# scipopt/SCIP-SDP

Hardware: AMD Instinct MI355X
Metric: node-SDP solves/sec, dense block n x n with m vars (IPM iters/sec in iters_per_sec) (higher is better)
Workload: dtype f64

## Files before the change

### include/hipsdp_units.h

```cpp
#ifndef HIPSDP_UNITS_H
#define HIPSDP_UNITS_H

#include "hipsdp.h"

#ifdef __cplusplus
extern "C" {
#endif

HIPSDP_API int  hipsdp_dgemm_selfcheck(int device, int M, int N, int K, int layB, int batch, int splitk, int flags, double beta,
   int* used_v2, long long* ndiff);
HIPSDP_API int  hipsdp_pass_at_unit(int device, int R, long long E, const double* A, const double* coef, double sa, const double* add, int split,
   double* out, int* chunks);
HIPSDP_API int  hipsdp_dgemm_selfcheck2(int device, int M, int N, int K, int layB, int batch, int splitk, int flags, double alpha, double beta,
   int reps, int* used, long long* ndiff, double* ms_tile, double* ms_fast);
HIPSDP_API int  hipsdp_gram_plan_info(int device, int M, long long K, int nslab, int* no, int* nd, int* nitems, double* span);
HIPSDP_API int  hipsdp_gram_selfcheck(int device, int M, long long K, int reps, int* used, double* maxdiff, long long* nrepro, double* ms_tile,
   double* ms_gram);
HIPSDP_API int  hipsdp_dgemm_selfcheck3(int device, int M, int N, int K, int layB, int batch, int splitk, int flags, double alpha, double beta,
   int reps, int* used, long long* ndiff, double* maxdiff, long long* nrepro, double* ms_tile, double* ms_fast);
HIPSDP_API int  hipsdp_schur_dense(int device, int m1, int n, const double* A, const double* X, const double* Zinv, double* Mx,
   double ws_gbytes);
HIPSDP_API int  hipsdp_schur_w(int device, int m1, int n, const double* A, const double* X, const double* Z, double* Mx);
HIPSDP_API int  hipsdp_schur_shard_time(int device, int m1, int n, int nranks, int rank, int by_columns, int reps, double ws_gbytes, double* ms);
HIPSDP_API int  hipsdp_schur_var_share_time(int device, int m1, int n, int nranks, int rank, int cw, int reps, double* ms, double* a2a_bytes);
HIPSDP_API int  hipsdp_schur_sparse_unit(int device, int n, int m, long long nnz, const int* var, const int* row, const int* col,
   const double* val, const double* X, const double* Zinv, double* Mx);
HIPSDP_API int  hipsdp_mfma_peak(int device, double ms, double* tflops, double* ghz);
HIPSDP_API int  hipsdp_potrf(int device, int n, double* A, int* fail);
HIPSDP_API int  hipsdp_potrf_ex(int device, int n, double* A, int psd, int v1, double* dinv, int* regmask, int* fail);
HIPSDP_API int  hipsdp_potrs(int device, int n, const double* A, int nrhs, double* rhs);
HIPSDP_API int  hipsdp_trtri(int device, int n, const double* A, double* Linv);
HIPSDP_API int  hipsdp_lambda_min(int device, int n, const double* W, int steps, double* theta, double* resid);
HIPSDP_API int  hipsdp_lambda_min_scaled(int device, int n, const double* L, const double* D, int steps, double* theta, double* resid);
HIPSDP_API int  hipsdp_solve1_fits(int m, int q, int nblk, const int* ns);
HIPSDP_API int  hipsdp_solve1_class(int m, int nblk, const int* ns);

#ifdef __cplusplus
}
#endif

#endif
```

### scip-sdp_amd/binding.py

```python
import ctypes as C
import os
import numpy as np

_HERE = os.path.dirname(os.path.abspath(__file__))
LIBPATH = os.environ.get("HIPSDP_LIB", os.path.join(_HERE, "lib", "libhipsdp.so"))

STATUS_NAMES = {0: "optimal", 1: "dual_infeasible", 2: "dual_unbounded", 3: "both_infeasible", 4: "iterlimit",
                5: "numeric", 6: "timelimit", 7: "objlimit", -1: "unsolved"}


class Params(C.Structure):
    _fields_ = [("gaptol", C.c_double), ("feastol", C.c_double), ("infeastol", C.c_double), ("objlimit", C.c_double),
                ("timelimit", C.c_double), ("gamma", C.c_double), ("ws_gbytes", C.c_double), ("maxiter", C.c_int),
                ("verbose", C.c_int), ("lanczos_steps", C.c_int), ("settings", C.c_int), ("pabstol", C.c_double), ("preoptgap", C.c_double)]


class Info(C.Structure):
    _fields_ = [("status", C.c_int), ("iterations", C.c_int), ("pobj", C.c_double), ("dobj", C.c_double),
                ("pinf", C.c_double), ("dinf", C.c_double), ("dabs", C.c_double), ("gap", C.c_double), ("mu", C.c_double),
                ("tau", C.c_double), ("kappa", C.c_double), ("solve_seconds", C.c_double), ("schur_seconds", C.c_double),
                ("schur_flops", C.c_double), ("schur_calls", C.c_int), ("chol_fail", C.c_int), ("warm_started", C.c_int),
                ("settings_used", C.c_int), ("schur_flops_executed", C.c_double)]


# ... 307 lines not shown
    col = np.ascontiguousarray(col, dtype=np.int32); val = _f64(val)
    X = _f64(X); Zinv = _f64(Zinv)
    Mx = np.zeros((m + 1, m + 1))
    _chk(ulib().hipsdp_schur_sparse_unit(device, n, m, C.c_longlong(len(val)), _ip(var), _ip(row), _ip(col), _dp(val), _dp(X), _dp(Zinv), _dp(Mx)),
         "hipsdp_schur_sparse_unit")
    return Mx


def schur_w(A, X, Z, device=0):
    A = _f64(A)
    m1, n = A.shape[0], A.shape[1]
    X = _f64(X)
    Z = _f64(Z)
    Mx = np.zeros((m1, m1))
    _chk(ulib().hipsdp_schur_w(device, m1, n, _dp(A), _dp(X), _dp(Z), _dp(Mx)), "hipsdp_schur_w")
    return Mx


def dgemm_selfcheck(M, N, K, layB=1, batch=1, splitk=1, flags=0, beta=0.0, device=0):
    used = C.c_int(0)
    nd = C.c_longlong(0)
    _chk(ulib().hipsdp_dgemm_selfcheck(device, M, N, K, layB, batch, splitk, flags, C.c_double(beta), C.byref(used), C.byref(nd)),
         "hipsdp_dgemm_selfcheck")
    return used.value, nd.value


def dgemm_selfcheck2(M, N, K, layB=1, batch=1, splitk=1, flags=0, alpha=1.0, beta=0.0, reps=0, device=0):
    used = C.c_int(0)
    nd = C.c_longlong(0)
    t0, t1 = C.c_double(0.0), C.c_double(0.0)
    _chk(ulib().hipsdp_dgemm_selfcheck2(device, M, N, K, layB, batch, splitk, flags, C.c_double(alpha), C.c_double(beta), reps,
                                       C.byref(used), C.byref(nd), C.byref(t0), C.byref(t1)), "hipsdp_dgemm_selfcheck2")
    return used.value, nd.value, t0.value, t1.value


def dgemm_selfcheck3(M, N, K, layB=1, batch=1, splitk=1, flags=0, alpha=1.0, beta=0.0, reps=0, device=0):
    used = C.c_int(0)
    nd, nr = C.c_longlong(0), C.c_longlong(0)
    md, t0, t1 = C.c_double(0.0), C.c_double(0.0), C.c_double(0.0)
    _chk(ulib().hipsdp_dgemm_selfcheck3(device, M, N, K, layB, batch, splitk, flags, C.c_double(alpha), C.c_double(beta), reps,
                                       C.byref(used), C.byref(nd), C.byref(md), C.byref(nr), C.byref(t0), C.byref(t1)), "hipsdp_dgemm_selfcheck3")
    return used.value, nd.value, md.value, nr.value, t0.value, t1.value


def gram_selfcheck(M, K, reps=0, device=0):
    used = C.c_int(0)
    nr = C.c_longlong(0)
    md, t0, t1 = C.c_double(0.0), C.c_double(0.0), C.c_double(0.0)
    _chk(ulib().hipsdp_gram_selfcheck(device, M, C.c_longlong(K), reps, C.byref(used), C.byref(md), C.byref(nr), C.byref(t0), C.byref(t1)),
         "hipsdp_gram_selfcheck")
    return used.value, md.value, nr.value, t0.value, t1.value


def potrf(A, device=0):
    L = _f64(A).copy()
    fail = C.c_int(0)
    _chk(ulib().hipsdp_potrf(device, L.shape[0], _dp(L), C.byref(fail)), "hipsdp_potrf")
    return np.tril(L), fail.value


def potrf_ex(A, psd=False, v1=False, device=0):
    L = _f64(A).copy()
    n = L.shape[0]
    dinv = np.zeros(((n + 63) // 64) * 4096)
    mask = np.zeros(n, dtype=np.int32)
    fail = C.c_int(0)
    _chk(ulib().hipsdp_potrf_ex(device, n, _dp(L), int(psd), int(v1), _dp(dinv), _ip(mask), C.byref(fail)), "hipsdp_potrf_ex")
    return L, dinv, mask, fail.value


def potrs(A, rhs, device=0):
    A = _f64(A)
    r = _f64(rhs).copy()
    r2 = r.reshape(-1, A.shape[0])
    _chk(ulib().hipsdp_potrs(device, A.shape[0], _dp(A), r2.shape[0], _dp(r2)), "hipsdp_potrs")
    return r2.reshape(r.shape)


def trtri(A, device=0):
    A = _f64(A)
    Li = np.zeros_like(A)
    _chk(ulib().hipsdp_trtri(device, A.shape[0], _dp(A), _dp(Li)), "hipsdp_trtri")
    return Li


def lambda_min(W, steps=0, device=0):
    W = _f64(W)
    th = C.c_double(0.0)
    rs = C.c_double(0.0)
    _chk(ulib().hipsdp_lambda_min(device, W.shape[0], _dp(W), steps, C.byref(th), C.byref(rs)), "hipsdp_lambda_min")
    return th.value, rs.value


def syev(A, device=0):
    A = _f64(A)
    n = A.shape[0]
    lam = np.zeros(n)
    V = np.zeros((n, n))
    _chk(lib().hipsdp_syev(device, n, _dp(A), _dp(lam), _dp(V)), "hipsdp_syev")
    return lam, V


def gemv_n(A, V, device=0):
    A = _f64(A)
    V = _f64(V).reshape(-1, A.shape[1])
    out = np.zeros((V.shape[0], A.shape[0]))
# ... 26 lines not shown
```

### scip-sdp_amd/csrc/hs_kernels.h

```cpp
#ifndef HS_KERNELS_H
#define HS_KERNELS_H

#include "hs_common.h"

int hs_fill(hipStream_t s, double* p, long long n, double v);
int hs_set_identity(hipStream_t s, double* A, int n, double v);
int hs_copy(hipStream_t s, double* dst, const double* src, long long n);
int hs_axpy(hipStream_t s, long long n, double a, const double* x, double* y);
int hs_scale_add(hipStream_t s, long long n, double a, const double* x, double b, const double* y, double* out);
int hs_mirror_lower(hipStream_t s, double* A, int n, long long lda);
int hs_symmetrize(hipStream_t s, double* A, int n);
int hs_transpose(hipStream_t s, int n, const double* src, double* dst);

int hs_gemv_n(hipStream_t s, int R, long long E, const double* A, long long lda, int nv, const double* const* V,
   double* out, long long ldo, double* ws, long long wsdoubles);
int hs_gemv_t(hipStream_t s, int R, long long E, const double* A, long long lda, const double* coef, double sa,
   const double* add, double* out);

int hs_gemv_t_chunks(int R, long long E);
int hs_gemv_t_ws(hipStream_t s, int R, long long E, const double* A, long long lda, const double* coef, double sa,
   const double* add, double* out, double* ws, long long wsdoubles);
int hs_gemv_t3(hipStream_t s, int R, long long E, const double* A, long long lda, const double* c0, const double* c1, const double* c2,
   double* o0, double* o1, double* o2);

void hs_red_batch_begin(hipStream_t s);
int hs_red_batch_end(void);
int hs_red_batch_end_publish(hipStream_t s, int n, const double* src, double* dst, unsigned long long seq, unsigned long long* flag);
void hs_red_batch_reset(void);
int hs_fill_scalar(hipStream_t s, double* p, double v);
int hs_red_batch_solve(hipStream_t s, int m, const double* dinv, const double* L, int nrhs, double* vec, long long ld);
struct hs_rb_finish { int m; double eta, rg, sigmu, tau, kappa, etk; const double* u1; const double* u2; double* dy; double* dyt; double* sc;
   int s0, bub, bh, wrp, bu1, dtau, dkappa, den; };
int hs_red_batch_finish(hipStream_t s, const void* fin, size_t bytes);
int hs_copy_scalar(hipStream_t s, double* dst, const double* src);
void hs_red_batch_hold(hipStream_t s);
int hs_red_batch_release(void);
int hs_red_batch_flush(void);
int hs_red_batch_end_all(void);
int hs_make_ext(hipStream_t s, int m, double s0, double s1, const double* v, double* ext);
int hs_lp_rows_small(hipStream_t s, int q, int m1, const double* Dext, const double* v, int mode, double eta, double sigmu, const double* x,
   const double* z, const double* rd, const double* elp, double* out1, double* out2);
#define HS_AS_MAXBLK 8
struct hs_as_args { int nblk; int n2[HS_AS_MAXBLK]; const double* A[HS_AS_MAXBLK]; const double* V[HS_AS_MAXBLK]; };
int hs_apply_A_small(hipStream_t s, int m1, const hs_as_args* B, int q, const double* Dext, const double* vlp, double* out, int epi,
   double scal, const double* vin, double* vout);
int hs_axpy3(hipStream_t s, double a, long long n1, const double* x1, double* y1, long long n2, const double* x2, double* y2,
   long long n3, const double* x3, double* y3);
int hs_dot(hipStream_t s, long long n, const double* a, const double* b, double* out, int accumulate, double* ws);
int hs_absmax(hipStream_t s, long long n, const double* a, double* out, int accumulate, double* ws);
int hs_ratio_min(hipStream_t s, long long n, const double* x, const double* d, double* out, int accumulate, double* ws);

#define HS_SMALL_N 48
int hs_dir_block_small(hipStream_t s, int n, double c, const double* X, const double* R, const double* E, const double* Zinv,
   double s1, double* out);
int hs_dirmat(hipStream_t s, int n, double s1, const double* Zinv, const double* X, const double* GZ, double* H);

int hs_lp_dir(hipStream_t s, int q, double sigmu, double eta, const double* x, const double* z, const double* rd_or_dz,
   const double* elp, double* out);
int hs_lp_scale_rows(hipStream_t s, int q, int cols, const double* x, const double* z, const double* D, double* S);
int hs_vec_mul(hipStream_t s, long long n, const double* a, const double* b, double* out);
int hs_lp_s0(hipStream_t s, int q, const double* x, const double* z, const double* beta, double* out, int accumulate, double* ws);

int hs_pack_rows(hipStream_t s, int m1, int n, long long Lp, const double* A, double* Apk);
int hs_pack_weighted(hipStream_t s, int n, const double* V, double* pk);
int hs_unpack_sym(hipStream_t s, int n, const double* pk, double sa, const double* add, double* out);
int hs_zero_upper(hipStream_t s, double* A, int n);

struct hs_schur_ws
{
   double*   T;
   double*   U;
   double*   K;
   double*   V;
   long long capT, capV;
   long long chunk_cols;
   long long n2;
   long long kws_len;
   int       full;
   double*   U2;
   double*   V2;
   void*     evP[2];
   void*     evX[2];
   void*     ev_g2;
   int       (*after_g1)(void*);
   void*     after_g1_arg;
};
int  hs_schur_ws_alloc(hs_schur_ws* w, int m1, long long n2max, double budget_gb);
void hs_schur_ws_free(hs_schur_ws* w);
int  hs_schur_U(hipStream_t s, int m1, int n, const double* A, const double* X, const double* Zinv, double* Mx,
   hs_schur_ws* w, int j_begin, int j_end);
int  hs_schur_W(hipStream_t s, int m1, int n, const double* A, const double* R, const double* G, double* Mx, hs_schur_ws* w);
int  hs_schur_W_identity(hipStream_t s, int m1, int n, const double* A, double* Mx, hs_schur_ws* w);
int  hs_schur_W_identity_range(hipStream_t s, int m1, int n, const double* A, long long k0, long long k1, double* Mx, hs_schur_ws* w);

int  hs_schur_Urows(hipStream_t s, int m1, int n, const double* A, const double* X, const double* Zinv, double* Mx,
   hs_schur_ws* w, int r_begin, int r_end);
void hs_shard_rows(int m1, int nranks, int rank, int* chunk_rows, int* first_begin, int* second_begin);
int  hs_schur_Wcols(hipStream_t s, int m1, int n, const double* A, const double* R, const double* G, double* Mx, hs_schur_ws* w,
   int c0, int cw);
void hs_shard_cols(int m1, int n, int nranks, int rank, int* c_begin, int* c_width);
int  hs_schur_Wvar(hipStream_t s, void* comm, int rank, int nranks, int m1, int n, const double* A, const double* R, const double* G,
   double* Mx, hs_schur_ws* w, int c0, int cw);
int  hs_schur_ws_alloc_var(hs_schur_ws* w, int m1, int nranks, int n, int cwmax);
int  hs_schur_ws_alloc_var_overlap(hs_schur_ws* w);
int  hs_schur_Wvar_all(hipStream_t s, hipStream_t sc, void* comm, int rank, int nranks, int m1, int n, const double* A, const double* R,
   const double* G, double* Mx, hs_schur_ws* w, int cwmax, int overlap);
void hs_var_rows(int m1, int nranks, int rank, int* r0, int* r1);
void hs_var_wrows(int n, int nranks, int rank, int* q0, int* q1);
int  hs_alltoall(void* comm, const double* send, double* recv, const long long* cnt, hipStream_t stream);
int  hs_allreduce_sum(void* comm, double* buf, long long count, hipStream_t stream);
int  hs_mirror_upper(hipStream_t s, double* A, int n, long long lda);
int  hs_allgather_inplace(void* comm, double* buf, long long count_per_rank, int rank, hipStream_t stream);
int  hs_allgather(void* comm, const double* send, double* recv, long long count_per_rank, hipStream_t stream);

struct hs_sparse;
int  hs_sp_prefers_sparse(int n, int m, long long nnz);
int  hs_sp_build(hs_sparse** out, int n, int m, long long nnz, const int* var, const int* row, const int* col, const double* val);
void hs_sp_free(hs_sparse* sp);
long long hs_sp_nnz(const hs_sparse* sp);
int  hs_sp_apply_A(hipStream_t s, const hs_sparse* sp, const double* V, double* out_var1);
int  hs_sp_apply_AT(hipStream_t s, const hs_sparse* sp, const double* coef, double* out);
int  hs_sp_schur(hipStream_t s, const hs_sparse* sp, const double* X, const double* Zinv, double* Mx);
int  hs_sp_expand(hipStream_t s, const hs_sparse* sp, double* A);

int hs_potrf(hipStream_t s, int n, double* A, double* dinv, int* flag, const double* diag0);
long long hs_potrf_dinv_len(int n);
int hs_potrf_psd(hipStream_t s, int n, double* A, double* dinv, int* flag, const double* diag0, int* regmask, int set_flag);
int hs_trtri(hipStream_t s, int n, const double* L, const double* dinv, double* Linv, double* tmp);
int hs_potrf_small_ext_pair(hipStream_t s, int n, double* const* L, double* const* dinv, int* const* flag, const double* const* base,
   const double* const* dir, double alpha, double* const* Mout, double* const* Linv, double* const* Gram, int set_flag);
int hs_potrf_small_ext(hipStream_t s, int n, double* L, double* dinv, int* flag, const double* base, const double* dir, double alpha,
   double* Mout, double* Linv, double* Gram, int set_flag);
int hs_schur_small(hipStream_t s, int m1, int nblk, const int* n, const double* const* A, const double* const* X,
   const double* const* Zinv, int q, const double* Dext, const double* x, const double* z, double* Mx, double* Lm, double* diagM);
int hs_trsv(hipStream_t s, int n, const double* L, const double* dinv, int nrhs, double* rhs, long long ldr, int mode);
long long hs_trsv_sync_ws(int n);
int hs_trsv_sync_init(hipStream_t s, int n, int* sync_ws, int* epoch);
int hs_trsv_sync(hipStream_t s, int n, const double* L, const double* dinv, int nrhs, double* rhs, long long ldr, int mode,
   int* sync_ws, int* epoch);

int hs_lanczos_lmin(hipStream_t s, int n, const double* W, int maxsteps, double* res, double* ws);
long long hs_lanczos_ws(int n, int maxsteps);
#define HS_STEP_MAXJOBS 32
struct hs_step_jobs { int nblk; int n[HS_STEP_MAXJOBS]; const double* L0[HS_STEP_MAXJOBS]; const double* D0[HS_STEP_MAXJOBS];
   const double* L1[HS_STEP_MAXJOBS]; const double* D1[HS_STEP_MAXJOBS]; double* res0[HS_STEP_MAXJOBS]; double* res1[HS_STEP_MAXJOBS]; };
int hs_steplen_small_multi(hipStream_t s, const hs_step_jobs* P, int maxsteps);
// ... 313 lines not shown
```

### scip-sdp_amd/csrc/ipm.hip

```cpp
#include "hs_kernels.h"
#include "../../include/hipsdp.h"
#include <rocprofiler-sdk-roctx/roctx.h>
#include <vector>
#include <utility>
#include <functional>
#include <chrono>
#include <algorithm>
#include <cmath>
#include <cstdio>
#include <cstdlib>
#include <cstring>

#define HS_LAUNCH_CHECK() do { hipError_t e_ = hipGetLastError(); if ( e_ != hipSuccess ) { hs_record_hip_error(e_, "kernel launch", __FILE__, __LINE__); return HS_ERR_HIP; } } while (0)

enum
{
   SC_AX0 = 0,
   SC_DOBJ,
   SC_XZ,
   SC_RP2,
   SC_RD2,
   SC_RDLPMAX,
   SC_HP2,
   SC_HD2,
   SC_S0,
   SC_BUB,
   SC_BH,
   SC_WRP,
   SC_BU1,
   SC_DTAU,
   SC_DKAPPA,
   SC_RATX,
   SC_RATZ,
   SC_DEN,
   SC_FIXED_END = 24
};
#define SC_BLK(k, i) (SC_FIXED_END + 8 * (k) + (i))

struct Block
{
   int     n;
   double* A;
   double* Aown;
   double* A0;
   double* A0sep;
   double* Apkown;
   double *X, *Z, *Rd, *Lz, *LzInv, *Zinv, *Lx, *LxInv, *B, *H, *G, *GZ, *dXa, *dZa, *dX, *dZ, *E, *W, *T1;
   double *dinvz, *dinvx;
   double *Xs, *Zs;
   double *T2, *W2;
   double *Xpre;
   double *P2;
   double *pk3;
   double *Apk;
   double *pkv;
   long long Lp;
   bool apk_valid;
   bool derived_valid;
   bool sparse;
   bool sp_dirty;
   hs_sparse* sp;
// ... 3197 lines not shown
               if ( identity_start && it == 0 )
               {
                  if ( g == g0 )
                  {
                     const long long n2 = (long long) B.n * B.n;
                     const int G = s->comm != NULL ? s->nranks : 1, r = s->comm != NULL ? s->rank : 0;
                     const long long k0 = ((n2 * r / G) / 8) * 8, k1 = r == G - 1 ? n2 : ((n2 * (r + 1) / G) / 8) * 8;
                     HS_CALL( hs_schur_W_identity_range(st, m1, B.n, B.A, k0, k1, s->Mx, &s->sws) );
                  }
                  gram_only_used = true;
                  continue;
               }
               HS_CALL( hs_schur_Wcols(st, m1, B.n, B.A, B.Lx, B.LzInv, s->Mx, &s->sws, c0, cw) );
            }
         if ( s->comm != NULL )
            HS_CALL( hs_allreduce_sum(s->comm, s->Mx, (long long) m1 * m1, st) );
      }
      else if ( s->comm != NULL || s->schur_mode_rows )
      {
         int c, b1, b2;
         hs_shard_rows(m1, s->nranks, s->rank, &c, &b1, &b2);
         for (auto& B : s->blk)
         {
            if ( B.sparse )
               continue;
            HS_CALL( hs_schur_Urows(st, m1, B.n, B.A, B.X, B.Zinv, s->Mx, &s->sws, b1, b1 + c) );
            HS_CALL( hs_schur_Urows(st, m1, B.n, B.A, B.X, B.Zinv, s->Mx, &s->sws, b2, b2 + c) );
         }
         if ( s->comm != NULL )
         {
            const long long cnt = (long long) c * m1;
            HS_CALL( hs_allgather_inplace(s->comm, s->Mx, cnt, s->rank, st) );
            HS_CALL( hs_allgather(s->comm, s->Mx + (long long) b2 * m1, s->Mgather, cnt, st) );
            for (int r = 0; r < s->nranks; ++r)
            {
               const long long dstrow = (long long) (2 * s->nranks - 1 - r) * c;
               if ( dstrow >= m1 )
                  continue;
               long long rowsleft = m1 - dstrow;
               if ( rowsleft > c ) rowsleft = c;
               HS_CALL( hs_copy(st, s->Mx + dstrow * m1, s->Mgather + (long long) r * cnt, rowsleft * m1) );
            }
         }
         HS_CALL( hs_mirror_upper(st, s->Mx, m1, m1) );
      }
      else
      {
         for (auto& B : s->blk)
         {
            if ( B.sparse )
               continue;
            if ( identity_start && it == 0 )
            {
               HS_CALL( hs_schur_W_identity(st, m1, B.n, B.A, s->Mx, &s->sws) );
               gram_only_used = true;
            }
            else if ( s->schur_mode_U )
               HS_CALL( hs_schur_U(st, m1, B.n, B.A, B.X, B.Zinv, s->Mx, &s->sws, 0, m1) );
            else
               HS_CALL( hs_schur_W(st, m1, B.n, B.A, B.Lx, B.LzInv, s->Mx, &s->sws) );
         }
      }
      for (auto& B : s->blk)
      {
         if ( !B.sparse )
            continue;
         const int n = B.n;
         HS_CALL( gemm(s, HS_KC, HS_MC, n, n, n, 1.0, B.X, n, B.A0, n, 0.0, B.T1, n) );
         HS_CALL( gemm(s, HS_KC, HS_MC, n, n, n, 1.0, B.T1, n, B.Zinv, n, 0.0, B.W, n) );
         HS_CALL( pass_A(s, B, B.W, s->tmpe) );
         hipLaunchKernelGGL(k_add_col0, g1d(m1), dim3(256), 0, st, m1, s->tmpe, s->Mx);
         HS_LAUNCH_CHECK();
         HS_CALL( hs_sp_schur(st, B.sp, B.X, B.Zinv, s->Mx) );
      }
      if ( q > 0 )
      {
         HS_CALL( hs_lp_scale_rows(st, q, m1, s->x, s->z, s->Dext, s->Slp) );
         HS_CALL( gemm(s, HS_MC, HS_MC, m1, m1, q, 1.0, s->Dext, m1, s->Slp, m1, 1.0, s->Mx, m1, HS_GEMM_LOWER) );
      }
      return hs_mirror_lower(st, s->Mx, m1, m1);
   }

   int solve_m()
   {
      phase_mark(s, PH_MSOLVE);
      predH_queued = predH_joined = split_dz = false;
      if ( s->use2 && s->comm == NULL && !small_problem(s) && m > 0 )
      {
         HS_CALL( fork2(s) );
         {
            QueueSwap sw(s);
            HS_CALL( direction(s, 0.0, 1.0, mu, rg, false, 0.0, 1) );
         }
         predH_queued = true;
      }
      if ( m > 0 )
      {
         if ( !schur_small )
         {
            HS_HIP( hipMemcpy2DAsync(s->Lm, (size_t) m * sizeof(double), s->Mx + m1 + 1, (size_t) m1 * sizeof(double),
                  (size_t) m * sizeof(double), (size_t) m, hipMemcpyDeviceToDevice, st) );
            HS_HIP( hipMemcpy2DAsync(s->dya, sizeof(double), s->Mx + m1 + 1, (size_t) (m1 + 1) * sizeof(double), sizeof(double), (size_t) m,
                  hipMemcpyDeviceToDevice, st) );
         }
         HS_CALL( hs_potrf_psd(st, m, s->Lm, s->dinvm, s->flags + 2, s->dya, s->regmask, setf) );
         if ( m <= 64 )
         {
// ... 965 lines not shown
```

### scip-sdp_amd/csrc/kernels.hip

```cpp
#include "hs_kernels.h"
#include <string.h>
#include <stdio.h>
#include <stdlib.h>

static int hs_rec_dir_block_small(hipStream_t s, int n, double c, const double* X, const double* R, const double* E, const double* Zinv,
   double s1, double* out);
static int hs_rec_lp_dir(hipStream_t s, int q, double sigmu, double eta, const double* x, const double* z, const double* r, const double* elp,
   double* out);
static int hs_rec_vec_mul(hipStream_t s, long long n, const double* a, const double* b, double* out);
static int hs_rec_axpy3(hipStream_t s, double a, long long n1, const double* x1, double* y1, long long n2, const double* x2, double* y2,
   long long n3, const double* x3, double* y3);
static int hs_rec_gemv_t(hipStream_t s, int R, long long E, const double* A, long long lda, const double* coef, double sa, const double* add,
   double* out);

struct __attribute__((aligned(16))) dbl2 { double x, y; };
__device__ __forceinline__ dbl2 load_stream2(const double* p)
{
   typedef double gv2 __attribute__((ext_vector_type(2)));
   const gv2 t = __builtin_nontemporal_load(reinterpret_cast<const gv2*>(p));
   dbl2 r; r.x = t.x; r.y = t.y;
   return r;
}

static inline int hs_launch_ok(void)
// ... 21 lines not shown
   }
}

__global__ void k_scale_add(long long n, double a, const double* __restrict__ x, double b, const double* __restrict__ y,
   double* __restrict__ out)
{
   for (long long i = (long long) blockIdx.x * blockDim.x + threadIdx.x; i < n; i += (long long) gridDim.x * blockDim.x)
   {
      double v = a * x[i];
      if ( y != NULL )
         v += b * y[i];
      out[i] = v;
   }
}

__global__ void k_mirror_lower(double* A, int n, long long lda)
{
   const long long total = (long long) n * n;
   for (long long i = (long long) blockIdx.x * blockDim.x + threadIdx.x; i < total; i += (long long) gridDim.x * blockDim.x)
   {
      const int r = (int) (i / n);
      const int c = (int) (i - (long long) r * n);
      if ( r < c )
         A[(long long) r * lda + c] = A[(long long) c * lda + r];
   }
}

__global__ void k_mirror_upper(double* A, int n, long long lda)
{
   const long long total = (long long) n * n;
   for (long long i = (long long) blockIdx.x * blockDim.x + threadIdx.x; i < total; i += (long long) gridDim.x * blockDim.x)
   {
      const int r = (int) (i / n);
      const int c = (int) (i - (long long) r * n);
      if ( r > c )
         A[(long long) r * lda + c] = A[(long long) c * lda + r];
   }
}

__global__ void k_pack_rows(int m1, int n, long long Lp, const double* __restrict__ A, double* __restrict__ Apk)
{
   const long long n2 = (long long) n * n;
   const long long total = (long long) m1 * n2;
   for (long long e = (long long) blockIdx.x * blockDim.x + threadIdx.x; e < total; e += (long long) gridDim.x * blockDim.x)
   {
      const long long i = e / n2;
      const long long rc = e - i * n2;
      const int r = (int) (rc / n), c = (int) (rc - (long long) r * n);
      if ( c <= r )
         Apk[i * Lp + (long long) r * (r + 1) / 2 + c] = A[e];
   }
}

__global__ void k_pack_weighted(int n, const double* __restrict__ V, double* __restrict__ pk)
{
   const long long total = (long long) n * n;
   for (long long e = (long long) blockIdx.x * blockDim.x + threadIdx.x; e < total; e += (long long) gridDim.x * blockDim.x)
   {
      const int r = (int) (e / n), c = (int) (e - (long long) (e / n) * n);
      if ( c <= r )
         pk[(long long) r * (r + 1) / 2 + c] = (r == c ? 1.0 : 2.0) * V[e];
   }
}

__global__ void k_unpack_sym(int n, const double* __restrict__ pk, double sa, const double* __restrict__ add, double* __restrict__ out)
{
   const long long total = (long long) n * n;
   for (long long e = (long long) blockIdx.x * blockDim.x + threadIdx.x; e < total; e += (long long) gridDim.x * blockDim.x)
   {
      const int r0 = (int) (e / n), c0 = (int) (e - (long long) (e / n) * n);
      const int r = r0 > c0 ? r0 : c0, c = r0 > c0 ? c0 : r0;
      double v = pk[(long long) r * (r + 1) / 2 + c];
      if ( add != NULL )
         v += sa * add[e];
      out[e] = v;
   }
}

__global__ void k_zero_upper(double* A, int n)
{
   const long long total = (long long) n * n;
   for (long long i = (long long) blockIdx.x * blockDim.x + threadIdx.x; i < total; i += (long long) gridDim.x * blockDim.x)
   {
      const int r = (int) (i / n);
      const int c = (int) (i - (long long) r * n);
      if ( r < c )
         A[i] = 0.0;
   }
}

__global__ void k_symmetrize(double* A, int n)
{
   const long long total = (long long) n * n;
   for (long long i = (long long) blockIdx.x * blockDim.x + threadIdx.x; i < total; i += (long long) gridDim.x * blockDim.x)
   {
      const int r = (int) (i / n);
      const int c = (int) (i - (long long) r * n);
      if ( r > c )
      {
         const double v = 0.5 * (A[(long long) r * n + c] + A[(long long) c * n + r]);
         A[(long long) r * n + c] = v;
         A[(long long) c * n + r] = v;
      }
   }
}

// ... 103 lines not shown

int hs_axpy3(hipStream_t s, double a, long long n1, const double* x1, double* y1, long long n2, const double* x2, double* y2,
   long long n3, const double* x3, double* y3)
{
   if ( n1 < 0 ) n1 = 0;
   if ( n2 < 0 ) n2 = 0;
   if ( n3 < 0 ) n3 = 0;
   if ( n1 + n2 + n3 == 0 ) return HS_OK;
   if ( hs_rec_axpy3(s, a, n1, x1, y1, n2, x2, y2, n3, x3, y3) )
      return HS_OK;
   hipLaunchKernelGGL(k_axpy3, dim3(grid_for(n1 + n2 + n3, 256, 2048)), dim3(256), 0, s, a, n1, x1, y1, n2, x2, y2, n3, x3, y3);
   HS_LAUNCH_CHECK();
   return HS_OK;
}

int hs_scale_add(hipStream_t s, long long n, double a, const double* x, double b, const double* y, double* out)
{
   (void) hs_red_batch_flush();
   if ( n <= 0 ) return HS_OK;
   hipLaunchKernelGGL(k_scale_add, dim3(grid_for(n, 256, 2048)), dim3(256), 0, s, n, a, x, b, y, out);
   HS_LAUNCH_CHECK();
   return HS_OK;
}

int hs_axpy(hipStream_t s, long long n, double a, const double* x, double* y)
{
   (void) hs_red_batch_flush();
   return hs_scale_add(s, n, a, x, 1.0, y, y);
}

int hs_mirror_lower(hipStream_t s, double* A, int n, long long lda)
{
   (void) hs_red_batch_flush();
   if ( n <= 1 ) return HS_OK;
   hipLaunchKernelGGL(k_mirror_lower, dim3(grid_for((long long) n * n, 256, 2048)), dim3(256), 0, s, A, n, lda);
   HS_LAUNCH_CHECK();
   return HS_OK;
}

int hs_mirror_upper(hipStream_t s, double* A, int n, long long lda)
{
   (void) hs_red_batch_flush();
   if ( n <= 1 ) return HS_OK;
   hipLaunchKernelGGL(k_mirror_upper, dim3(grid_for((long long) n * n, 256, 2048)), dim3(256), 0, s, A, n, lda);
   HS_LAUNCH_CHECK();
   return HS_OK;
}

int hs_pack_rows(hipStream_t s, int m1, int n, long long Lp, const double* A, double* Apk)
{
   (void) hs_red_batch_flush();
   HS_HIP( hipMemsetAsync(Apk, 0, (size_t) m1 * (size_t) Lp * sizeof(double), s) );
   hipLaunchKernelGGL(k_pack_rows, dim3(grid_for((long long) m1 * n * n, 256, 65536)), dim3(256), 0, s, m1, n, Lp, A, Apk);
   HS_LAUNCH_CHECK();
   return HS_OK;
}

int hs_pack_weighted(hipStream_t s, int n, const double* V, double* pk)
{
   (void) hs_red_batch_flush();
   hipLaunchKernelGGL(k_pack_weighted, dim3(grid_for((long long) n * n, 256, 2048)), dim3(256), 0, s, n, V, pk);
   HS_LAUNCH_CHECK();
   return HS_OK;
}

int hs_unpack_sym(hipStream_t s, int n, const double* pk, double sa, const double* add, double* out)
{
   (void) hs_red_batch_flush();
   hipLaunchKernelGGL(k_unpack_sym, dim3(grid_for((long long) n * n, 256, 2048)), dim3(256), 0, s, n, pk, sa, add, out);
   HS_LAUNCH_CHECK();
   return HS_OK;
}

int hs_zero_upper(hipStream_t s, double* A, int n)
{
   (void) hs_red_batch_flush();
   if ( n <= 1 ) return HS_OK;
   hipLaunchKernelGGL(k_zero_upper, dim3(grid_for((long long) n * n, 256, 2048)), dim3(256), 0, s, A, n);
   HS_LAUNCH_CHECK();
   return HS_OK;
}

__global__ void __launch_bounds__(256) k_transpose(int n, const double* __restrict__ src, double* __restrict__ dst)
{
   __shared__ double tile[32][33];
   const int bx = blockIdx.x * 32, by = blockIdx.y * 32;
   const int tx = threadIdx.x & 31, ty = threadIdx.x >> 5;
   for (int r = ty; r < 32; r += 8)
      if ( by + r < n && bx + tx < n )
         tile[r][tx] = src[(long long) (by + r) * n + bx + tx];
   __syncthreads();
   for (int r = ty; r < 32; r += 8)
      if ( bx + r < n && by + tx < n )
         dst[(long long) (bx + r) * n + by + tx] = tile[tx][r];
}

int hs_transpose(hipStream_t s, int n, const double* src, double* dst)
{
   (void) hs_red_batch_flush();
   if ( n <= 0 ) return HS_OK;
   const int t = (n + 31) / 32;
   hipLaunchKernelGGL(k_transpose, dim3(t, t), dim3(256), 0, s, n, src, dst);
   HS_LAUNCH_CHECK();
   return HS_OK;
}

// ... 1710 lines not shown
```

### scip-sdp_amd/csrc/schur.hip

```cpp
#include "hs_kernels.h"
#include "hs_lds_product.h"
#include <vector>
#include <cmath>
#include <stdlib.h>

int hs_schur_ws_alloc(hs_schur_ws* w, int m1, long long n2max, double budget_gb)
{
   w->T = w->U = w->K = w->V = w->U2 = w->V2 = NULL;
   w->evP[0] = w->evP[1] = w->evX[0] = w->evX[1] = NULL;
   w->ev_g2 = NULL;
   w->after_g1 = NULL; w->after_g1_arg = NULL;
   w->capT = w->capV = 0;
   const double need_full = 2.0 * 8.0 * (double) m1 * (double) n2max;
   long long cols = m1;
   w->full = 1;
   if ( need_full > budget_gb * 1e9 )
   {
      w->full = 0;
      cols = (long long) (budget_gb * 1e9 / (2.0 * 8.0 * (double) n2max));
      cols = (cols / 128) * 128;
      if ( cols < 128 ) cols = 128;
      if ( cols > m1 ) cols = m1;
   }
   w->chunk_cols = cols;
// ... 17 lines not shown
   w->kws_len = (long long) sk * m1 * (w->full ? m1 : cols);
   e = hs_pool_alloc((void**) &w->K, (size_t) w->kws_len * sizeof(double)) == HS_OK ? hipSuccess : hipErrorOutOfMemory;
   if ( e != hipSuccess )
   {
      hs_record_hip_error(e, "hipMalloc(split-K slabs)", __FILE__, __LINE__);
      return e == hipErrorOutOfMemory ? HS_ERR_NOMEM : HS_ERR_HIP;
   }
   return HS_OK;
}

void hs_schur_ws_free(hs_schur_ws* w)
{
   hs_pool_free(w->T);
   hs_pool_free(w->U);
   hs_pool_free(w->K);
   hs_pool_free(w->V);
   hs_pool_free(w->U2);
   hs_pool_free(w->V2);
   for (int i = 0; i < 2; ++i)
   {
      if ( w->evP[i] != NULL ) (void) hipEventDestroy((hipEvent_t) w->evP[i]);
      if ( w->evX[i] != NULL ) (void) hipEventDestroy((hipEvent_t) w->evX[i]);
      w->evP[i] = w->evX[i] = NULL;
   }
   w->T = w->U = w->K = w->V = w->U2 = w->V2 = NULL;
}

int hs_schur_U(hipStream_t s, int m1, int n, const double* A, const double* X, const double* Zinv, double* Mx,
   hs_schur_ws* w, int j_begin, int j_end)
{
   const long long n2 = (long long) n * n;
   if ( n2 > 2000000000LL )
      return HS_ERR_ARG;
   for (int j0 = j_begin; j0 < j_end; j0 += (int) w->chunk_cols)
   {
      const int cj = (j_end - j0) < w->chunk_cols ? (j_end - j0) : (int) w->chunk_cols;
      const long long rows = (long long) cj * n;
      if ( rows > 2000000000LL )
         return HS_ERR_ARG;
      hs_gemm_args g1 = {(int) rows, n, n, HS_KC, HS_MC, A + (long long) j0 * n2, n, 0, Zinv, n, 0, w->T, n, 0, 1.0, 0.0, 1, HS_GEMM_REMAP, 1, NULL};
      HS_CALL( hs_dgemm(s, &g1) );
      hs_gemm_args g2 = {n, n, n, HS_KC, HS_MC, X, n, 0, w->T, n, n2, w->U, n, n2, 1.0, 0.0, cj, HS_GEMM_REMAP, 1, NULL};
      HS_CALL( hs_dgemm(s, &g2) );
      const int rowsM = m1 - j0;
      int sk = hs_dgemm_pick_splitk(rowsM, cj, (int) n2, 1);
      while ( sk > 1 && (long long) sk * rowsM * cj > w->kws_len ) --sk;
      hs_gemm_args g3 = {rowsM, cj, (int) n2, HS_KC, HS_KC, A + (long long) j0 * n2, n2, 0, w->U, n2, 0,
         Mx + (long long) j0 * m1 + j0, m1, 0, 1.0, 1.0, 1, HS_GEMM_LOWER, sk, w->K};
      HS_CALL( hs_dgemm(s, &g3) );
   }
   return HS_OK;
}

static int schur_gram(hipStream_t s, int m1, long long K, const double* V, long long ldv, double* Mx, hs_schur_ws* w, int* done)
{
   *done = 0;
   long long nslab = w->kws_len / ((long long) m1 * m1);
   if ( nslab > 64 ) nslab = 64;
   double executed = 0.0;
   const int r = hs_gram_try(s, m1, K, V, ldv, Mx, m1, 1.0, 1.0, w->K, (int) nslab, &executed);
   if ( r < 0 )
      return -r;
   if ( r == 1 )
   {
      hs_mfma_flops_add(executed);
      *done = 1;
   }
   return HS_OK;
}

#define SYRK_MIN_M1 256

static void schur_syrk_shape(const hs_schur_ws* w, int m1, long long K, bool xcd, int* flags, int* sk)
{
   const long long slab = (long long) m1 * m1;
   *flags = HS_GEMM_LOWER;
   if ( xcd && 2 * slab <= w->kws_len )
   {
      const long long tm = (m1 + 127) / 128;
      int s = hs_dgemm_pick_xcd_slices(tm * (tm + 1) / 2, K);
      if ( s < 2 ) s = 2;
      while ( s > 2 && (long long) s * slab > w->kws_len ) --s;
      *sk = s;
      *flags |= HS_GEMM_XCD | HS_GEMM_NOFAST;
      return;
   }
   int s = hs_dgemm_pick_splitk(m1, m1, (int) K, 1);
   while ( s > 1 && (long long) s * slab > w->kws_len ) --s;
   *sk = s < 1 ? 1 : s;
}

int hs_schur_W_identity_range(hipStream_t s, int m1, int n, const double* A, long long k0, long long k1, double* Mx, hs_schur_ws* w)
{
   const long long n2 = (long long) n * n;
   const long long K = k1 - k0;
   if ( n2 > 2000000000LL || k0 < 0 || k1 > n2 || (k0 & 1) )
      return HS_ERR_ARG;
   if ( K <= 0 )
      return HS_OK;
   {
      int done = 0;
      HS_CALL( schur_gram(s, m1, K, A + k0, n2, Mx, w, &done) );
      if ( done )
         return HS_OK;
   }
   int flags, sk;
   schur_syrk_shape(w, m1, K, m1 >= SYRK_MIN_M1 && K >= 16384 && (K >= 50000 || m1 >= 900), &flags, &sk);
   hs_gemm_args g3 = {m1, m1, (int) K, HS_KC, HS_KC, A + k0, n2, 0, A + k0, n2, 0, Mx, m1, 0, 1.0, 1.0, 1, flags, sk, sk > 1 ? w->K : NULL};
   return hs_dgemm(s, &g3);
}

int hs_schur_W_identity(hipStream_t s, int m1, int n, const double* A, double* Mx, hs_schur_ws* w)
{
   return hs_schur_W_identity_range(s, m1, n, A, 0, (long long) n * n, Mx, w);
}

int hs_schur_W(hipStream_t s, int m1, int n, const double* A, const double* R, const double* G, double* Mx, hs_schur_ws* w)
{
   const long long n2 = (long long) n * n;
   const long long rows = (long long) m1 * n;
   if ( !w->full || n2 > 2000000000LL || rows > 2000000000LL )
      return HS_ERR_ARG;
   hs_gemm_args g1 = {(int) rows, n, n, HS_KC, HS_MC, A, n, 0, R, n, 0, w->T, n, 0, 1.0, 0.0, 1, HS_GEMM_B_LOWTRI, 1, NULL};
   HS_CALL( hs_dgemm(s, &g1) );
   if ( w->after_g1 != NULL )
   {
      int (*f)(void*) = w->after_g1;
      w->after_g1 = NULL;
      HS_CALL( f(w->after_g1_arg) );
   }
   if ( w->ev_g2 != NULL )
      HS_HIP( hipStreamWaitEvent(s, (hipEvent_t) w->ev_g2, 0) );
   hs_gemm_args g2 = {n, n, n, HS_KC, HS_MC, G, n, 0, w->T, n, n2, w->U, n, n2, 1.0, 0.0, m1, HS_GEMM_A_LOWTRI | HS_GEMM_REMAP, 1, NULL};
   HS_CALL( hs_dgemm(s, &g2) );
   {
      int done = 0;
      HS_CALL( schur_gram(s, m1, n2, w->U, n2, Mx, w, &done) );
      if ( done )
         return HS_OK;
   }
   int flags = HS_GEMM_LOWER;
   int sk;
   if ( m1 >= SYRK_MIN_M1 && n2 >= 16384 && (n2 >= 50000 || m1 >= 900) )
   {
      const long long tm = (m1 + 127) / 128;
      const long long ntri = tm * (tm + 1) / 2;
      sk = hs_dgemm_pick_xcd_slices(ntri, n2);
      while ( sk > 2 && (long long) sk * m1 * m1 > w->kws_len ) --sk;
      flags |= HS_GEMM_XCD;
      flags |= HS_GEMM_NOFAST;
   }
   else
   {
      sk = hs_dgemm_pick_splitk(m1, m1, (int) n2, 1);
      while ( sk > 1 && (long long) sk * m1 * m1 > w->kws_len ) --sk;
   }
   hs_gemm_args g3 = {m1, m1, (int) n2, HS_KC, HS_KC, w->U, n2, 0, w->U, n2, 0, Mx, m1, 0, 1.0, 1.0, 1, flags, sk, w->K};
   HS_CALL( hs_dgemm(s, &g3) );
   return HS_OK;
}

int hs_schur_Wcols(hipStream_t s, int m1, int n, const double* A, const double* R, const double* G, double* Mx, hs_schur_ws* w,
   int c0, int cw)
{
   if ( cw <= 0 )
      return HS_OK;
   const long long rows = (long long) m1 * n;
// ... 434 lines not shown
```

### scip-sdp_amd/csrc/units.hip

```cpp
#include "hs_kernels.h"
#include "../../include/hipsdp.h"
#include "../../include/hipsdp_units.h"
#include <vector>
#include <cstring>
#include <cstdlib>

namespace {

struct DevBuf
{
   double* p;
   DevBuf() : p(NULL) {}
   ~DevBuf() { if ( p ) (void) hipFree(p); }
   int alloc(long long n) { if ( n <= 0 ) n = 1; hipError_t e = hipMalloc((void**) &p, (size_t) n * sizeof(double)); if ( e != hipSuccess ) { hs_record_hip_error(e, "hipMalloc", __FILE__, __LINE__); return e == hipErrorOutOfMemory ? HS_ERR_NOMEM : HS_ERR_HIP; } return HS_OK; }
   int up(const double* h, long long n) { if ( n <= 0 ) return HS_OK; hipError_t e = hipMemcpy(p, h, (size_t) n * sizeof(double), hipMemcpyHostToDevice); if ( e != hipSuccess ) { hs_record_hip_error(e, "H2D", __FILE__, __LINE__); return HS_ERR_HIP; } return HS_OK; }
   int down(double* h, long long n) { if ( n <= 0 ) return HS_OK; hipError_t e = hipMemcpy(h, p, (size_t) n * sizeof(double), hipMemcpyDeviceToHost); if ( e != hipSuccess ) { hs_record_hip_error(e, "D2H", __FILE__, __LINE__); return HS_ERR_HIP; } return HS_OK; }
};

int pick_device(int device)
{
   int nd = 0;
   if ( hipGetDeviceCount(&nd) != hipSuccess || nd <= 0 )
      return HIPSDP_ERR_NODEVICE;
   if ( device < 0 || device >= nd )
// ... 261 lines not shown
   }
   *used = r2 == 1 ? 1 : 0;
   *maxdiff = 0.0; *nrepro = 0;
   unsigned long long h[2] = {0, 0};
   if ( rc == HS_OK && r2 == 1 )
   {
      if ( hipMemset(dn, 0, 2 * sizeof(unsigned long long)) != hipSuccess ) rc = HS_ERR_HIP;
      hipLaunchKernelGGL(k_unit_lowdiff, dim3(1024), dim3(256), 0, 0, M, dC1.p, dC2.p, dn);
      if ( rc == HS_OK && hipMemcpy(h, dn, sizeof(h), hipMemcpyDeviceToHost) != hipSuccess ) rc = HS_ERR_HIP;
      memcpy(maxdiff, &h[0], sizeof(double));
      if ( rc == HS_OK && hipMemset(dn, 0, 2 * sizeof(unsigned long long)) != hipSuccess ) rc = HS_ERR_HIP;
      hipLaunchKernelGGL(k_unit_lowdiff, dim3(1024), dim3(256), 0, 0, M, dC2.p, dC3.p, dn);
      if ( rc == HS_OK && hipMemcpy(h, dn, sizeof(h), hipMemcpyDeviceToHost) != hipSuccess ) rc = HS_ERR_HIP;
      *nrepro = (long long) h[1];
   }
   if ( rc == HS_OK && reps > 0 && ms_tile != NULL && ms_gram != NULL )
   {
      hipEvent_t e0, e1;
      HS_HIP( hipEventCreate(&e0) ); HS_HIP( hipEventCreate(&e1) );
      for (int which = 0; which < 2 && rc == HS_OK; ++which)
      {
         for (int it = -2; it < reps && rc == HS_OK; ++it)
         {
            if ( it == 0 )
               (void) hipEventRecord(e0, 0);
            if ( which == 0 )
               rc = hs_dgemm(0, &g3);
            else if ( r2 == 1 )
            {
               const int r = hs_gram_try(0, M, K, dW.p, K, dC2.p, M, 1.0, 1.0, dS.p, nslab, &ex);
               if ( r < 0 ) rc = -r;
            }
         }
         (void) hipEventRecord(e1, 0);
         float t = 0.f;
         if ( rc == HS_OK && (hipEventSynchronize(e1) != hipSuccess || hipEventElapsedTime(&t, e0, e1) != hipSuccess) )
            rc = HS_ERR_HIP;
         *(which == 0 ? ms_tile : ms_gram) = (double) t / reps;
      }
      (void) hipEventDestroy(e0); (void) hipEventDestroy(e1);
   }
   if ( rc == HS_OK && hipDeviceSynchronize() != hipSuccess )
      rc = HS_ERR_HIP;
   (void) hipFree(dn);
   return rc;
}

extern "C" int hipsdp_gram_plan_info(int device, int M, long long K, int nslab, int* no, int* nd, int* nitems, double* span)
{
   HS_CALL( pick_device(device) );
   return hs_gram_plan_info(M, K, nslab, no, nd, nitems, span) ? HIPSDP_OK : HIPSDP_ERR_ARG;
}

extern "C" int hipsdp_schur_dense(int device, int m1, int n, const double* A, const double* X, const double* Zinv, double* Mx,
   double ws_gbytes)
{
   HS_CALL( pick_device(device) );
   const long long n2 = (long long) n * n;
   DevBuf dA, dX, dZ, dM;
   HS_CALL( dA.alloc(m1 * n2) ); HS_CALL( dX.alloc(n2) ); HS_CALL( dZ.alloc(n2) ); HS_CALL( dM.alloc((long long) m1 * m1) );
   HS_CALL( dA.up(A, m1 * n2) ); HS_CALL( dX.up(X, n2) ); HS_CALL( dZ.up(Zinv, n2) );
   hs_schur_ws w;
   HS_CALL( hs_schur_ws_alloc(&w, m1, n2, ws_gbytes > 0.0 ? ws_gbytes : 1e9) );
   if ( ws_gbytes > 0.0 && w.chunk_cols > 1 )
   {
      long long cols = (long long) (ws_gbytes * 1e9 / (16.0 * (double) n2));
      if ( cols < 1 ) cols = 1;
      if ( cols < w.chunk_cols ) w.chunk_cols = cols;
   }
   HS_CALL( hs_fill(0, dM.p, (long long) m1 * m1, 0.0) );
   int rc = hs_schur_U(0, m1, n, dA.p, dX.p, dZ.p, dM.p, &w, 0, m1);
   if ( rc == HS_OK ) rc = hs_mirror_lower(0, dM.p, m1, m1);
   if ( rc == HS_OK && hipDeviceSynchronize() != hipSuccess ) rc = HS_ERR_HIP;
   hs_schur_ws_free(&w);
   HS_CALL( rc );
   HS_CALL( dM.down(Mx, (long long) m1 * m1) );
   return HIPSDP_OK;
}

extern "C" int hipsdp_schur_shard_time(int device, int m1, int n, int nranks, int rank, int by_columns, int reps, double ws_gbytes,
   double* ms)
{
   HS_CALL( pick_device(device) );
   if ( m1 < 1 || n < 1 || nranks < 1 || rank < 0 || rank >= nranks || reps < 1 || ms == NULL )
      return HIPSDP_ERR_ARG;
   const long long n2 = (long long) n * n;
   DevBuf dA, dX, dZ, dM;
   HS_CALL( dA.alloc(m1 * n2) ); HS_CALL( dX.alloc(n2) ); HS_CALL( dZ.alloc(n2) ); HS_CALL( dM.alloc((long long) (m1 + 32) * m1) );
   hipLaunchKernelGGL(k_unit_fill, dim3(1024), dim3(256), 0, 0, m1 * n2, 11ULL, dA.p);
   hipLaunchKernelGGL(k_unit_fill, dim3(1024), dim3(256), 0, 0, n2, 23ULL, dX.p);
   hipLaunchKernelGGL(k_unit_fill, dim3(1024), dim3(256), 0, 0, n2, 37ULL, dZ.p);
   hs_schur_ws w;
   int c, b1, b2, c0 = 0, cw = 0;
   hs_shard_rows(m1, nranks, rank, &c, &b1, &b2);
   hs_shard_cols(m1, n, nranks, rank, &c0, &cw);
   HS_CALL( hs_schur_ws_alloc(&w, m1, by_columns ? (long long) n * (cw > 0 ? cw : 1) : n2, ws_gbytes > 0.0 ? ws_gbytes : 40.0) );
   hipEvent_t e0, e1;
   HS_HIP( hipEventCreate(&e0) ); HS_HIP( hipEventCreate(&e1) );
   int rc = HS_OK;
   for (int it = 0; it <= reps && rc == HS_OK; ++it)
   {
      if ( it == 1 )
         rc = hipEventRecord(e0, 0) == hipSuccess ? HS_OK : HS_ERR_HIP;
      if ( rc == HS_OK ) rc = hs_fill(0, dM.p, (long long) m1 * m1, 0.0);
      if ( by_columns )
      {
// ... 386 lines not shown
```

Measured before the change: 12.48.

## Compute identity-start Schur Gram from packed triangular storage with diagonal correction

For the first IPM iteration with identity start, the Schur matrix is now formed from the packed lower-triangle rows (about n(n+1)/2 instead of n^2 entries per constraint). It scales the packed Gram product by 2 and subtracts a small diagonal-only product to recover the full trace inner products. This roughly halves the K dimension of the dominant SYRK/Gram, at the cost of an extra small GEMM, a diagonal extraction kernel and a lower-triangle subtraction. It only applies when packed data exists and the workspace fits, and it affects only iteration 0.

```diff
diff --git a/include/hipsdp_units.h b/include/hipsdp_units.h
--- a/include/hipsdp_units.h
+++ b/include/hipsdp_units.h
@@ -18,6 +18,8 @@
    double* ms_gram);
 HIPSDP_API int  hipsdp_dgemm_selfcheck3(int device, int M, int N, int K, int layB, int batch, int splitk, int flags, double alpha, double beta,
    int reps, int* used, long long* ndiff, double* maxdiff, long long* nrepro, double* ms_tile, double* ms_fast);
+HIPSDP_API int  hipsdp_schur_identity_unit(int device, int m1, int n, const double* A, double ws_gbytes, int full_storage, double* Mx,
+   double* flops);
 HIPSDP_API int  hipsdp_schur_dense(int device, int m1, int n, const double* A, const double* X, const double* Zinv, double* Mx,
    double ws_gbytes);
 HIPSDP_API int  hipsdp_schur_w(int device, int m1, int n, const double* A, const double* X, const double* Z, double* Mx);
diff --git a/scip-sdp_amd/binding.py b/scip-sdp_amd/binding.py
--- a/scip-sdp_amd/binding.py
+++ b/scip-sdp_amd/binding.py
@@ -383,6 +383,16 @@
     return used.value, md.value, nr.value, t0.value, t1.value
 
 
+def schur_identity_unit(A, Mx=None, ws_gbytes=0.0, full_storage=False, device=0):
+    A = _f64(A)
+    m1, n = A.shape[0], A.shape[1]
+    Mx = np.zeros((m1, m1)) if Mx is None else _f64(Mx).copy()
+    fl = C.c_double(0.0)
+    _chk(ulib().hipsdp_schur_identity_unit(device, m1, n, _dp(A), C.c_double(ws_gbytes), int(full_storage), _dp(Mx), C.byref(fl)),
+         "hipsdp_schur_identity_unit")
+    return Mx, fl.value
+
+
 def potrf(A, device=0):
     L = _f64(A).copy()
     fail = C.c_int(0)
diff --git a/scip-sdp_amd/csrc/hs_kernels.h b/scip-sdp_amd/csrc/hs_kernels.h
--- a/scip-sdp_amd/csrc/hs_kernels.h
+++ b/scip-sdp_amd/csrc/hs_kernels.h
@@ -62,6 +62,8 @@
 int hs_lp_s0(hipStream_t s, int q, const double* x, const double* z, const double* beta, double* out, int accumulate, double* ws);
 
 int hs_pack_rows(hipStream_t s, int m1, int n, long long Lp, const double* A, double* Apk);
+int hs_packed_diag(hipStream_t s, int m1, int n, int ldd, long long Lp, const double* Apk, double* D);
+int hs_sub_lower(hipStream_t s, int n, const double* S, double* C);
 int hs_pack_weighted(hipStream_t s, int n, const double* V, double* pk);
 int hs_unpack_sym(hipStream_t s, int n, const double* pk, double sa, const double* add, double* out);
 int hs_zero_upper(hipStream_t s, double* A, int n);
@@ -92,6 +94,8 @@
 int  hs_schur_W(hipStream_t s, int m1, int n, const double* A, const double* R, const double* G, double* Mx, hs_schur_ws* w);
 int  hs_schur_W_identity(hipStream_t s, int m1, int n, const double* A, double* Mx, hs_schur_ws* w);
 int  hs_schur_W_identity_range(hipStream_t s, int m1, int n, const double* A, long long k0, long long k1, double* Mx, hs_schur_ws* w);
+int  hs_schur_W_identity_packed(hipStream_t s, int m1, int n, const double* Apk, long long Lp, double* Mx, hs_schur_ws* w);
+int  hs_schur_identity_packed_fits(const hs_schur_ws* w, int m1, int n);
 
 int  hs_schur_Urows(hipStream_t s, int m1, int n, const double* A, const double* X, const double* Zinv, double* Mx,
    hs_schur_ws* w, int r_begin, int r_end);
diff --git a/scip-sdp_amd/csrc/ipm.hip b/scip-sdp_amd/csrc/ipm.hip
--- a/scip-sdp_amd/csrc/ipm.hip
+++ b/scip-sdp_amd/csrc/ipm.hip
@@ -7,6 +7,7 @@
 #include <chrono>
 #include <algorithm>
 #include <cmath>
+#include <cassert>
 #include <cstdio>
 #include <cstdlib>
 #include <cstring>
@@ -3310,7 +3311,11 @@
                continue;
             if ( identity_start && it == 0 )
             {
-               HS_CALL( hs_schur_W_identity(st, m1, B.n, B.A, s->Mx, &s->sws) );
+               assert(B.Apk == NULL || B.apk_valid);
+               if ( B.Apk != NULL && hs_schur_identity_packed_fits(&s->sws, m1, B.n) )
+                  HS_CALL( hs_schur_W_identity_packed(st, m1, B.n, B.Apk, B.Lp, s->Mx, &s->sws) );
+               else
+                  HS_CALL( hs_schur_W_identity(st, m1, B.n, B.A, s->Mx, &s->sws) );
                gram_only_used = true;
             }
             else if ( s->schur_mode_U )
diff --git a/scip-sdp_amd/csrc/kernels.hip b/scip-sdp_amd/csrc/kernels.hip
--- a/scip-sdp_amd/csrc/kernels.hip
+++ b/scip-sdp_amd/csrc/kernels.hip
@@ -97,6 +97,28 @@
    }
 }
 
+__global__ void k_packed_diag(int m1, int n, int ldd, long long Lp, const double* __restrict__ Apk, double* __restrict__ D)
+{
+   const long long total = (long long) m1 * ldd;
+   for (long long e = (long long) blockIdx.x * blockDim.x + threadIdx.x; e < total; e += (long long) gridDim.x * blockDim.x)
+   {
+      const long long i = e / ldd;
+      const int r = (int) (e - i * ldd);
+      D[e] = r < n ? Apk[i * Lp + (long long) r * (r + 3) / 2] : 0.0;
+   }
+}
+
+__global__ void k_sub_lower(int n, const double* __restrict__ S, double* __restrict__ C)
+{
+   const long long total = (long long) n * n;
+   for (long long e = (long long) blockIdx.x * blockDim.x + threadIdx.x; e < total; e += (long long) gridDim.x * blockDim.x)
+   {
+      const int r = (int) (e / n), c = (int) (e - (long long) r * n);
+      if ( c <= r )
+         C[e] -= S[e];
+   }
+}
+
 __global__ void k_pack_weighted(int n, const double* __restrict__ V, double* __restrict__ pk)
 {
    const long long total = (long long) n * n;
@@ -306,6 +328,24 @@
    (void) hs_red_batch_flush();
    HS_HIP( hipMemsetAsync(Apk, 0, (size_t) m1 * (size_t) Lp * sizeof(double), s) );
    hipLaunchKernelGGL(k_pack_rows, dim3(grid_for((long long) m1 * n * n, 256, 65536)), dim3(256), 0, s, m1, n, Lp, A, Apk);
+   HS_LAUNCH_CHECK();
+   return HS_OK;
+}
+
+int hs_packed_diag(hipStream_t s, int m1, int n, int ldd, long long Lp, const double* Apk, double* D)
+{
+   (void) hs_red_batch_flush();
+   if ( ldd < n )
+      return HS_ERR_ARG;
+   hipLaunchKernelGGL(k_packed_diag, dim3(grid_for((long long) m1 * ldd, 256, 2048)), dim3(256), 0, s, m1, n, ldd, Lp, Apk, D);
+   HS_LAUNCH_CHECK();
+   return HS_OK;
+}
+
+int hs_sub_lower(hipStream_t s, int n, const double* S, double* C)
+{
+   (void) hs_red_batch_flush();
+   hipLaunchKernelGGL(k_sub_lower, dim3(grid_for((long long) n * n, 256, 2048)), dim3(256), 0, s, n, S, C);
    HS_LAUNCH_CHECK();
    return HS_OK;
 }
diff --git a/scip-sdp_amd/csrc/schur.hip b/scip-sdp_amd/csrc/schur.hip
--- a/scip-sdp_amd/csrc/schur.hip
+++ b/scip-sdp_amd/csrc/schur.hip
@@ -93,13 +93,13 @@
    return HS_OK;
 }
 
-static int schur_gram(hipStream_t s, int m1, long long K, const double* V, long long ldv, double* Mx, hs_schur_ws* w, int* done)
+static int schur_gram(hipStream_t s, int m1, long long K, const double* V, long long ldv, double* Mx, hs_schur_ws* w, int* done, double alpha = 1.0)
 {
    *done = 0;
    long long nslab = w->kws_len / ((long long) m1 * m1);
    if ( nslab > 64 ) nslab = 64;
    double executed = 0.0;
-   const int r = hs_gram_try(s, m1, K, V, ldv, Mx, m1, 1.0, 1.0, w->K, (int) nslab, &executed);
+   const int r = hs_gram_try(s, m1, K, V, ldv, Mx, m1, alpha, 1.0, w->K, (int) nslab, &executed);
    if ( r < 0 )
       return -r;
    if ( r == 1 )
@@ -154,6 +154,33 @@
 int hs_schur_W_identity(hipStream_t s, int m1, int n, const double* A, double* Mx, hs_schur_ws* w)
 {
    return hs_schur_W_identity_range(s, m1, n, A, 0, (long long) n * n, Mx, w);
+}
+
+int hs_schur_identity_packed_fits(const hs_schur_ws* w, int m1, int n)
+{
+   return w->T != NULL && (long long) m1 * ((n + 1) & ~1) <= w->chunk_cols * w->n2;
+}
+
+int hs_schur_W_identity_packed(hipStream_t s, int m1, int n, const double* Apk, long long Lp, double* Mx, hs_schur_ws* w)
+{
+   const int ldd = (n + 1) & ~1;
+   if ( n < 1 || Lp < (long long) n * (n + 1) / 2 || (Lp & 1) || Lp > 2000000000LL || !hs_schur_identity_packed_fits(w, m1, n) )
+      return HS_ERR_ARG;
+   int done = 0;
+   HS_CALL( schur_gram(s, m1, Lp, Apk, Lp, Mx, w, &done, 2.0) );
+   if ( !done )
+   {
+      int flags, sk;
+      schur_syrk_shape(w, m1, Lp, m1 >= SYRK_MIN_M1 && Lp >= 16384 && (Lp >= 50000 || m1 >= 900), &flags, &sk);
+      hs_gemm_args g3 = {m1, m1, (int) Lp, HS_KC, HS_KC, Apk, Lp, 0, Apk, Lp, 0, Mx, m1, 0, 2.0, 1.0, 1, flags, sk, sk > 1 ? w->K : NULL};
+      HS_CALL( hs_dgemm(s, &g3) );
+   }
+   HS_CALL( hs_packed_diag(s, m1, n, ldd, Lp, Apk, w->T) );
+   const bool slab = w->K != NULL && (long long) m1 * m1 <= w->kws_len;
+   hs_gemm_args gd = {m1, m1, n, HS_KC, HS_KC, w->T, ldd, 0, w->T, ldd, 0, slab ? w->K : Mx, m1, 0, slab ? 1.0 : -1.0, slab ? 0.0 : 1.0, 1,
+      HS_GEMM_LOWER, 1, NULL};
+   HS_CALL( hs_dgemm(s, &gd) );
+   return slab ? hs_sub_lower(s, m1, w->K, Mx) : HS_OK;
 }
 
 int hs_schur_W(hipStream_t s, int m1, int n, const double* A, const double* R, const double* G, double* Mx, hs_schur_ws* w)
diff --git a/scip-sdp_amd/csrc/units.hip b/scip-sdp_amd/csrc/units.hip
--- a/scip-sdp_amd/csrc/units.hip
+++ b/scip-sdp_amd/csrc/units.hip
@@ -337,6 +337,43 @@
    return hs_gram_plan_info(M, K, nslab, no, nd, nitems, span) ? HIPSDP_OK : HIPSDP_ERR_ARG;
 }
 
+extern "C" int hipsdp_schur_identity_unit(int device, int m1, int n, const double* A, double ws_gbytes, int full_storage, double* Mx,
+   double* flops)
+{
+   HS_CALL( pick_device(device) );
+   if ( m1 <= 0 || n <= 0 || A == NULL || Mx == NULL )
+      return HIPSDP_ERR_ARG;
+   const long long n2 = (long long) n * n;
+   const long long Lp = (((long long) n * (n + 1) / 2) + 1) & ~1LL;
+   DevBuf dA, dP, dM;
+   HS_CALL( dA.alloc(m1 * n2) ); HS_CALL( dM.alloc((long long) m1 * m1) );
+   HS_CALL( dA.up(A, m1 * n2) ); HS_CALL( dM.up(Mx, (long long) m1 * m1) );
+   if ( !full_storage )
+      HS_CALL( dP.alloc(m1 * Lp) );
+   hs_schur_ws w;
+   int rc = hs_schur_ws_alloc(&w, m1, n2, ws_gbytes > 0.0 ? ws_gbytes : 40.0);
+   if ( rc != HS_OK )
+   {
+      hs_schur_ws_free(&w);
+      return rc;
+   }
+   const double before = hs_mfma_flops_total();
+   if ( full_storage )
+      rc = hs_schur_W_identity(0, m1, n, dA.p, dM.p, &w);
+   else
+   {
+      rc = hs_pack_rows(0, m1, n, Lp, dA.p, dP.p);
+      if ( rc == HS_OK ) rc = hs_schur_W_identity_packed(0, m1, n, dP.p, Lp, dM.p, &w);
+   }
+   if ( flops != NULL )
+      *flops = hs_mfma_flops_total() - before;
+   if ( rc == HS_OK && hipDeviceSynchronize() != hipSuccess ) rc = HS_ERR_HIP;
+   hs_schur_ws_free(&w);
+   HS_CALL( rc );
+   HS_CALL( dM.down(Mx, (long long) m1 * m1) );
+   return HIPSDP_OK;
+}
+
 extern "C" int hipsdp_schur_dense(int device, int m1, int n, const double* A, const double* X, const double* Zinv, double* Mx,
    double ws_gbytes)
 {
```

New measurement: 12.83 (median of 6 runs). +2.7%, better.
